# zackLiuzz/MY_ORB_SLAM2

Measured on AMD Instinct MI355X. Metric: frames/sec ORB extract+match, KITTI 1241×376 stereo, 1/2/4/8 GPU, higher is better.
Workload: dtype u8

## Files before the change

### my_orb_slam2_amd/csrc/orbx_capi.hip

```cpp
#include <hip/hip_runtime.h>

#include <algorithm>
#include <chrono>
#include <condition_variable>
#include <cfloat>
#include <climits>
#include <cmath>
#include <cstdio>
#include <cstdlib>
#include <cstring>
#include <functional>
#include <map>
#include <memory>
#include <mutex>
#include <shared_mutex>
#include <thread>
#include <vector>

#include "../../include/orbx.h"
#include "orbx_internal.h"
#include "orbx_kernels.h"

#ifndef ORBX_SRC_HASH
#define ORBX_SRC_HASH "0000000000000000"
// ... 143 lines not shown
        h->sigma2[i] = h->scale[i] * h->scale[i];
    }
    for (int i = 0; i < L; i++) {
        h->inv_scale[i] = 1.0f / h->scale[i];
        h->inv_sigma2[i] = 1.0f / h->sigma2[i];
    }
    const int nfeatures = h->prm.nfeatures;
    float factor = (float)(1.0f / scaleFactor);
    float nDesired = nfeatures * (1 - factor) / (1 - (float)pow((double)factor, (double)L));
    int sum = 0;
    for (int level = 0; level < L - 1; level++) {
        h->nfeat[level] = cvRound(nDesired);
        sum += h->nfeat[level];
        nDesired *= factor;
    }
    h->nfeat[L - 1] = std::max(nfeatures - sum, 0);
    const int HP = 15;
    int v, v0, vmax = cvFloor((float)(HP * std::sqrt(2.f) / 2 + 1));
    int vmin = cvCeil((float)(HP * std::sqrt(2.f) / 2));
    const double hp2 = HP * HP;
    for (v = 0; v <= vmax; ++v) h->umax[v] = cvRound(std::sqrt(hp2 - v * v));
    for (v = HP, v0 = 0; v >= vmin; --v) {
        while (h->umax[v0] == h->umax[v0 + 1]) ++v0;
        h->umax[v] = v0;
        ++v0;
    }
    float cf[7];
    double s2 = -0.5 / (2.0 * 2.0), ksum = 0;
    for (int i = 0; i < 7; ++i) {
        double x = i - 3.0;
        cf[i] = (float)std::exp(s2 * x * x);
        ksum += cf[i];
    }
    ksum = 1. / ksum;
    for (int i = 0; i < 7; ++i) cf[i] = (float)(cf[i] * ksum);
    for (int i = 0; i < 7; ++i) h->taps[i] = cvRound(cf[i] * 256.f);
}

int reflect101_h(int p, int len) {
    if ((unsigned)p < (unsigned)len) return p;
    if (len == 1) return 0;
    do {
        if (p < 0) p = -p;
        else p = 2 * len - 2 - p;
    } while ((unsigned)p >= (unsigned)len);
    return p;
}

void reflected_range_h(int lo, int hi, int len, int& mn, int& mx) {
    mn = 1 << 30;
    mx = -1;
    for (int p = lo; p <= hi; ++p) {
        const int r = reflect101_h(p, len);
        mn = std::min(mn, r);
        mx = std::max(mx, r);
    }
}

int vresize_simd_end(int width) {
    int x = 0;
    for (; x <= width - 16; x += 16) {}
    for (; x < width - 4; x += 4) {}
    return x;
}

static int strip_default(const LevelGeom& lv, int nimg, int ncu) {
    const long long target = 2LL * ncu * 4;
    int th = STRIP_TH;
    while (th > 8 && (long long)lv.snw * ((lv.h + th - 1) / th) * nimg < target) th /= 2;
    return th;
}

static void strip_heights(const orbx_extractor* h, int nimg, int* sth) {
    for (int l = 0; l < ORBX_MAX_LEVELS; ++l) sth[l] = STRIP_TH;
    for (int l = 0; l < h->hg.nlevels; ++l) {
        const LevelGeom& lv = h->hg.lv[l];
        if (lv.strip) sth[l] = strip_default(lv, nimg, h->ncu);
    }
}

static int stereo_split_of(int pairs) { return orbx::stereo_split(pairs); }

#define OCT_LDS_SMALL_KB 152
#define OCT_SMALL_BATCH 16
#define CHAIN_MAX_BATCH 8
#define SIDE_MIN_BATCH 16

static int fast_cells_per_wave(int ncells, int batch, int ncu) {
    int nc = FAST_NC;
    while (nc > 1 && (long long)ncells * batch / (4 * nc) < 2LL * ncu) nc >>= 1;
    return nc;
}

static int octree_small(int batch) { return batch <= OCT_SMALL_BATCH ? 1 : 0; }
static int side_mode_of(const orbx_extractor* h, int batch) {
    return (h->side_auto && batch < SIDE_MIN_BATCH) ? 0 : h->side_mode;
}
static int chain_of(const orbx_extractor* h, int in_place, int side_mode, int batch) {
    return (h->hg.chain_ok && in_place && side_mode == 0 && batch <= CHAIN_MAX_BATCH) ? 1 : 0;
}

static std::shared_mutex g_capture_mu;

static bool order_after_last(orbx_extractor* h, hipStream_t st) {
    if (h->have_done && h->done_stream != st) {
        std::shared_lock<std::shared_mutex> lk(g_capture_mu);
        return HIPOK(hipStreamWaitEvent(st, h->done, 0));
    }
    return true;
}

static bool mark_done(orbx_extractor* h, hipStream_t st) {
    h->done_stream = st;
    h->have_done = true;
    return HIPOK(hipEventRecord(h->done, st));
}

static bool wait_idle(orbx_extractor* h) {
    return !h->have_done || HIPOK(hipEventSynchronize(h->done));
}

#define WAIT_SPIN_US 400
static bool wait_done(orbx_extractor* h) {
    const int spin_us = WAIT_SPIN_US;
    if (spin_us > 0) {
        const auto t0 = std::chrono::steady_clock::now();
        for (;;) {
            const hipError_t e = hipEventQuery(h->done);
            if (e == hipSuccess) return true;
            if (e != hipErrorNotReady) return HIPOK(e);
            if (std::chrono::steady_clock::now() - t0 > std::chrono::microseconds(spin_us)) break;
            std::this_thread::yield();
        }
    }
    return HIPOK(hipEventSynchronize(h->done));
}

static bool ensure_pinned(uint8_t*& p, size_t& cap, size_t n) {
    if (p && cap >= n) return true;
    if (p) (void)hipHostFree(p);
    p = nullptr;
    cap = 0;
    if (!HIPOK(hipHostMalloc((void**)&p, n, hipHostMallocDefault))) { p = nullptr; return false; }
    cap = n;
    return true;
}

void build_strip_tables(orbx_extractor* h, int l, int mode, const int16_t* xofs,
                        const int16_t* alpha, const int16_t* yofs, const int16_t* beta) {
    Geometry& G = h->hg;
    LevelGeom& lv = G.lv[l];
    lv.strip = 0;
    if (mode != 0 && mode != 3) return;
    const LevelGeom& S = G.lv[l > 0 ? l - 1 : 0];
    lv.snh = (lv.w + SW_PX - 1) / SW_PX;
    lv.snw = (lv.snh + 1) / 2;
    std::vector<StripLane> sl((size_t)lv.snh * 32);
    for (int hs = 0; hs < lv.snh; ++hs)
        for (int q = 0; q < 32; ++q) {
            StripLane& e = sl[(size_t)hs * 32 + q];
            memset(&e, 0, sizeof(e));
            int xr[4];
            const int xg = hs * SW_PX - 4 + 4 * q;
            for (int j = 0; j < 4; ++j)
                xr[j] = xg > lv.w + 3 ? lv.w - 1 : reflect101_h(xg + j, lv.w);
            if (mode == 0) {
                const int mn = std::min(std::min(xr[0], xr[1]), std::min(xr[2], xr[3]));
                e.base = (uint32_t)mn;
                for (int j = 0; j < 4; ++j) {
                    if (xr[j] - mn > 4) return;
                    e.sel |= (uint32_t)(xr[j] - mn) << (8 * j);
                }
            } else {
                int sx[4];
                for (int j = 0; j < 4; ++j) sx[j] = xofs[xr[j]];
                const int mn = std::min(std::min(sx[0], sx[1]), std::min(sx[2], sx[3]));
                e.base = (uint32_t)mn;
                for (int j = 0; j < 4; ++j) {
                    const int k = sx[j] - mn;
                    if (k > 6) return;
                    e.psel[j] = (uint32_t)k | (0x0Cu << 8) | ((uint32_t)(k + 1) << 16) | (0x0Cu << 24);
                    uint32_t a0 = (uint16_t)alpha[2 * xr[j]], a1 = (uint16_t)alpha[2 * xr[j] + 1];
                    if (xr[j] >= lv.xmax) { a0 = 2048; a1 = 0; }
                    e.alp[j] = (a0 << 4) | ((a1 << 4) << 16);
                    e.flags |= (uint32_t)((xr[j] < lv.xmax ? 1 : 0) | (xr[j] < lv.rsimd_end ? 2 : 0))
                               << (2 * j);
                }
            }
        }
    std::vector<uint32_t> rt((size_t)4 * (lv.h + 6));
    for (int k = 0; k < lv.h + 6; ++k) {
        const int yr = reflect101_h(k - 3, lv.h);
        if (mode == 0) {
            rt[4 * k] = (uint32_t)yr;
        } else {
            const int sy = yofs[yr];
            const uint32_t r0 = (uint32_t)std::min(std::max(sy, 0), S.h - 1);
            const uint32_t r1 = (uint32_t)std::min(std::max(sy + 1, 0), S.h - 1);
            rt[4 * k] = r0 * (uint32_t)S.pitch;
            rt[4 * k + 1] = r1 * (uint32_t)S.pitch;
            rt[4 * k + 2] = (uint32_t)(uint16_t)beta[2 * yr] | ((uint32_t)(uint16_t)beta[2 * yr + 1] << 16);
        }
    }
    h->ltab.resize(align_up(h->ltab.size(), 16));
    lv.stab = (int)h->ltab.size();
    h->ltab.insert(h->ltab.end(), (const uint8_t*)sl.data(), (const uint8_t*)(sl.data() + sl.size()));
    h->ltab.resize(align_up(h->ltab.size(), 16));
    lv.srow = (int)h->ltab.size();
    h->ltab.insert(h->ltab.end(), (const uint8_t*)rt.data(), (const uint8_t*)(rt.data() + rt.size()));
    h->ltab.resize(align_up(h->ltab.size(), 16));
    lv.strip = 1;
}

static void build_chain(orbx_extractor* h) {
    Geometry& G = h->hg;
    const int L = G.nlevels;
    G.chain_ok = 0;
    G.chain_gx = G.chain_gy = 1;
    G.chain_tab = G.chain_toffs = 0;
    G.chain_buf = G.chain_rs = G.chain_lds = 0;
    for (int l = 1; l < L; ++l) {
        if (G.lv[l].copy || G.lv[l].area2) return;
        const int16_t* xofs = h->rtab.data() + G.lv[l].rtab_off;
        for (int x = 0; x < G.lv[l].w; x += 4)
            if (xofs[std::min(x + 3, G.lv[l].w - 1)] - xofs[x] > 5) return;
    }
    const int gx = std::max(1, (G.lv[0].w + CHAIN_TW - 1) / CHAIN_TW);
    const int gy = std::max(1, (G.lv[0].h + CHAIN_TH - 1) / CHAIN_TH);
    std::vector<ChainRect> rects((size_t)gx * gy * L);
    std::vector<int32_t> toffs((size_t)gx * gy * 2 * (L + 1), 0);
    size_t buf = 16, rs = 16, ct = 16;
    for (int ty = 0; ty < gy; ++ty)
        for (int tx = 0; tx < gx; ++tx) {
            size_t tab = 0;
            bool have_next = false;
            int nx0 = 0, nx1 = -1, ny0 = 0, ny1 = -1;
            for (int l = L - 1; l >= 0; --l) {
                const LevelGeom& lv = G.lv[l];
                const int W = lv.w, Hh = lv.h;
                const int ox0 = tx == 0 ? 0 : ((int)((long long)tx * W / gx) & ~3);
                const int ox1 = std::max(ox0, tx == gx - 1 ? W : ((int)((long long)(tx + 1) * W / gx) & ~3));
                const int oy0 = (int)((long long)ty * Hh / gy);
                const int oy1 = std::max(oy0, ty == gy - 1 ? Hh : (int)((long long)(ty + 1) * Hh / gy));
                int fx0 = INT_MAX, fx1 = -1, fy0 = INT_MAX, fy1 = -1;
                if (ox1 > ox0 && oy1 > oy0) {
                    fx0 = std::max(ox0 - 3, 0);
                    fx1 = std::min(ox1 + 2, W - 1);
                    fy0 = std::max(oy0 - 3, 0);
                    fy1 = std::min(oy1 + 2, Hh - 1);
                }
                if (have_next) {
                    const LevelGeom& D = G.lv[l + 1];
                    const int16_t* xofs = h->rtab.data() + D.rtab_off;
                    const int16_t* yofs = xofs + 3 * D.w;
                    fx0 = std::min(fx0, std::min(std::max((int)xofs[nx0], 0), W - 1));
                    fx1 = std::max(fx1, std::min((int)xofs[nx1] + 1, W - 1));
                    fy0 = std::min(fy0, std::min(std::max((int)yofs[ny0], 0), Hh - 1));
                    fy1 = std::max(fy1, std::min(std::max((int)yofs[ny1] + 1, 0), Hh - 1));
                }
                ChainRect& c = rects[((size_t)ty * gx + tx) * L + l];
                c.ox0 = (int16_t)ox0;
                c.ox1 = (int16_t)ox1;
                c.oy0 = (int16_t)oy0;
                c.oy1 = (int16_t)oy1;
                if (fx1 < 0) {
                    c.fx0 = c.fy0 = 0;
                    c.fx1 = c.fy1 = -1;
                    have_next = false;
                    continue;
                }
                fx0 &= ~3;
                c.fx0 = (int16_t)fx0;
                c.fx1 = (int16_t)fx1;
                c.fy0 = (int16_t)fy0;
                c.fy1 = (int16_t)fy1;
                have_next = true;
                nx0 = fx0;
                nx1 = fx1;
                ny0 = fy0;
                ny1 = fy1;
                const int fw = fx1 - fx0 + 1;
                buf = std::max(buf, (size_t)chain_pitch(fw) * (fy1 - fy0 + 1) + 16);
                rs = std::max(rs, (size_t)4 * ((ox1 - ox0 + 3) & ~3) * (oy1 - oy0 + 6));
                if (l > 0) tab += chain_level_words((fw + 3) >> 2, fy1 - fy0 + 1);
            }
            ct = std::max(ct, 4 * tab);
            int32_t* te = &toffs[((size_t)ty * gx + tx) * 2 * (L + 1)];
            int32_t* tw = te + (L + 1);
            for (int l = 1; l < L; ++l) {
                const ChainRect& c = rects[((size_t)ty * gx + tx) * L + l];
                const int fw = c.fx1 - c.fx0 + 1, fh = c.fy1 - c.fy0 + 1;
                te[l + 1] = te[l] + (fw > 0 ? ((fw + 3) >> 2) + ((fh + 1) & ~1) : 0);
                tw[l + 1] = tw[l] + (fw > 0 ? chain_level_words((fw + 3) >> 2, fh) : 0);
            }
        }
    auto r16 = [](size_t v) { return (v + 15) & ~(size_t)15; };
    const size_t lds = 2 * r16(buf) + r16(rs) + r16(ct);
    if (lds > 150 * 1024) return;
    G.chain_gx = gx;
    G.chain_gy = gy;
    G.chain_buf = (int)r16(buf);
    G.chain_rs = (int)r16(rs);
    G.chain_lds = (int)lds;
    while (h->ltab.size() % 16) h->ltab.push_back(0);
    G.chain_tab = (int)h->ltab.size();
    h->ltab.insert(h->ltab.end(), (const uint8_t*)rects.data(), (const uint8_t*)(rects.data() + rects.size()));
    while (h->ltab.size() % 16) h->ltab.push_back(0);
    G.chain_toffs = (int)h->ltab.size();
    h->ltab.insert(h->ltab.end(), (const uint8_t*)toffs.data(), (const uint8_t*)(toffs.data() + toffs.size()));
    G.chain_ok = 1;
}

orbx_status build_geometry(orbx_extractor* h, int W, int H) {
    Geometry& G = h->hg;
    memset(&G, 0, sizeof(G));
    for (int i = 0; i < 3; ++i)
        if (h->taps[i] != h->taps[6 - i]) return ORBX_ERR_UNSUPPORTED;
    h->cells.clear();
    h->rtab.clear();
    const int L = h->prm.nlevels;
    G.width = W;
    G.height = H;
    G.nlevels = L;
    G.ini_th = std::min(std::max(h->prm.ini_th_fast, 0), 255);
    G.min_th = std::min(std::max(h->prm.min_th_fast, 0), 255);
    memcpy(G.taps, h->taps, sizeof(G.taps));
    memcpy(G.umax, h->umax, sizeof(G.umax));
    for (int l = 0; l < L; ++l)
        G.lv[l].stereo_win = (int)std::ceil(2.0f * h->scale[l]) + 2;
    long long off = 0, cand = 0;
    int out = 0, blur_tiles = 0, oblocks = 0;
    for (int l = 0; l < L; ++l) {
        LevelGeom& lv = G.lv[l];
        lv.w = cvRound((float)W * h->inv_scale[l]);
        lv.h = cvRound((float)H * h->inv_scale[l]);
        if (lv.w <= 0 || lv.h <= 0) return ORBX_ERR_UNSUPPORTED;
        if (lv.w > 4096 + 32 || lv.h > 4096 + 32) return ORBX_ERR_UNSUPPORTED;
        lv.pitch = (int)align_up(lv.w + 4, 64);
        lv.off = off;
        off += (long long)align_up((size_t)lv.pitch * align_up((size_t)lv.h, 4), 256);
        lv.scale = h->scale[l];
        lv.inv_scale = h->inv_scale[l];
        lv.nfeat = h->nfeat[l];
        lv.patch_size = (int)(31 * h->scale[l]);
        const int minB = ORBX_MIN_BORDER;
        const int maxBX = lv.w - ORBX_EDGE + 3, maxBY = lv.h - ORBX_EDGE + 3;
        const float width = (float)(maxBX - minB), height = (float)(maxBY - minB);
        const int nCols = (int)(width / 30.f), nRows = (int)(height / 30.f);
        lv.ncols = nCols;
        lv.nrows = nRows;
        lv.cell_begin = (int)h->cells.size();
        lv.cand_off = cand;
        int lcap = 0;
        if (nCols > 0 && nRows > 0) {
// ... 1522 lines not shown
```

### my_orb_slam2_amd/csrc/orbx_pyramid.hip

```cpp
#include <hip/hip_runtime.h>
#include <stdint.h>

#include <type_traits>
#include <utility>

#include "orbx_device.h"
#include "orbx_internal.h"
#include "orbx_kernels.h"

namespace orbx {


#define LT_GW (LT_W / 4)

__device__ __forceinline__ int reflect101_i(int p, int len) {
    if ((unsigned)p < (unsigned)len) return p;
    if (len == 1) return 0;
    do {
        if (p < 0) p = -p;
        else p = 2 * len - 2 - p;
    } while ((unsigned)p >= (unsigned)len);
    return p;
}

// ... 380 lines not shown
            const uint32_t wa0 = __builtin_amdgcn_alignbyte(a1, a0, o0);
            const uint32_t wa1 = __builtin_amdgcn_alignbyte(a2, a1, o0);
            const uint32_t wc0 = __builtin_amdgcn_alignbyte(c1, c0, o0);
            const uint32_t wc1 = __builtin_amdgcn_alignbyte(c2, c1, o0);
            const bool all_simd = FASTP || ((ci >> 1) & 0x55u) == 0x55u;
            auto hsum = [&](int j, int& h0, int& h1) {
                const uint32_t p0 = __builtin_amdgcn_perm(wa1, wa0, sels[j]);
                const uint32_t p1 = __builtin_amdgcn_perm(wc1, wc0, sels[j]);
                const us2 al = __builtin_bit_cast(us2, als[j]);
                h0 = (int)__builtin_amdgcn_udot2(__builtin_bit_cast(us2, p0), al, 0u, false);
                h1 = (int)__builtin_amdgcn_udot2(__builtin_bit_cast(us2, p1), al, 0u, false);
            };
            const uint32_t bs0 = (uint32_t)b0 << 8, bs1 = (uint32_t)b1 << 8;
            auto mulhi24 = [](uint32_t x, uint32_t y) {
                return (uint32_t)(((uint64_t)(x & 0xFFFFFFu) * (y & 0xFFFFFFu)) >> 32);
            };
            auto vsimd = [&](int H0, int H1) {
                return (int)((mulhi24((uint32_t)H0 & ~0xFFu, bs0) +
                              mulhi24((uint32_t)H1 & ~0xFFu, bs1) + 2u) >> 2);
            };
            if (all_simd) {
#pragma unroll
                for (int j = 0; j < 4; ++j) {
                    int h0, h1;
                    hsum(j, h0, h1);
                    out |= (uint32_t)vsimd(h0, h1) << (8 * j);
                }
            } else {
#pragma unroll
                for (int j = 0; j < 4; ++j) {
                    int h0, h1;
                    hsum(j, h0, h1);
                    const int vs = vsimd(h0, h1);
                    h0 >>= 4;
                    h1 >>= 4;
                    const int vc = min((int)((__umul24(h0, b0) + __umul24(h1, b1) + (1u << 21)) >> 22), 255);
                    out |= (uint32_t)(((ci >> (2 * j + 1)) & 1u) ? vs : vc) << (8 * j);
                }
            }
        } else {
#pragma unroll
            for (int j = 0; j < 4; ++j) {
                const int sxj = xs[j];
                const int f = (int)(ci >> (2 * j)) & 3;
                int h0, h1;
                if (f & 1) {
                    const int aa = (int)(int16_t)(als[j] & 0xFFFF), ab = (int)(int16_t)(als[j] >> 16);
                    h0 = w0[sxj] * aa + w0[sxj + 1] * ab;
                    h1 = w1[sxj] * aa + w1[sxj + 1] * ab;
                } else {
                    h0 = w0[sxj] * 2048;
                    h1 = w1[sxj] * 2048;
                }
                out |= (uint32_t)vresize(h0, h1, b0, b1, (f & 2) != 0) << (8 * j);
            }
        }
        return out;
    };
    auto level_item = [&](int hr, int q, bool all) {
        const int y = Y0 - 3 + hr, xg = X0 - 4 + 4 * q;
        uint32_t out = 0;
        if (all || (y >= ny0 && y <= ny1 && xg + 3 >= nx0 && xg <= nx1)) {
            const uint2 cg = cgrp[q];
            const uint32_t ci = cinf[q];
            const uint2 ri = rinf[hr];
            const int xs[4] = {(int)(cg.x & 0xFFFF), (int)(cg.x >> 16), (int)(cg.y & 0xFFFF),
                               (int)(cg.y >> 16)};
            if (mode == 3) {
                out = item3(hr, cg, ci, calp[q], csel[q], std::false_type{});
            } else if (mode == 2) {
                const int yr = (int)ri.x;
#pragma unroll
                for (int j = 0; j < 4; ++j) {
                    const uint8_t* s0 = src2 + (size_t)(2 * yr) * S.pitch + 2 * xs[j];
                    out |= (uint32_t)((s0[0] + s0[1] + s0[S.pitch] + s0[S.pitch + 1] + 2) >> 2) << (8 * j);
                }
            } else {
                const uint8_t* wr = win + __umul24(ri.x & 0xFFFF, WP);
                if (ci & 0x100u) {
                    out = *(const uint32_t*)(wr + xs[0]);
                } else {
                    out = (uint32_t)wr[xs[0]] | ((uint32_t)wr[xs[1]] << 8) |
                          ((uint32_t)wr[xs[2]] << 16) | ((uint32_t)wr[xs[3]] << 24);
                }
            }
        }
        lvl[hr * LT_G + q] = out;
    };
    if (!direct && mode == 3 && full_tile) {
        if (tid < 7 * LT_G) {
            const int rs = (int)(__umul24((uint32_t)tid, 1928u) >> 16);
            const int q = tid - rs * LT_G;
            const uint2 cg = cgrp[q];
            const uint32_t ci = cinf[q];
            const uint4 al = calp[q], sl = csel[q];
            const bool fast = (ci & 0x200u) && ((ci >> 1) & 0x55u) == 0x55u;
            if (__all(fast)) {
#pragma unroll
                for (int k = 0; k < (LT_HR + 6) / 7; ++k) {
                    const int hr = rs + 7 * k;
                    if (hr < LT_HR) lvl[hr * LT_G + q] = item3(hr, cg, ci, al, sl, std::true_type{});
                }
            } else {
#pragma unroll
                for (int k = 0; k < (LT_HR + 6) / 7; ++k) {
                    const int hr = rs + 7 * k;
                    if (hr < LT_HR) lvl[hr * LT_G + q] = item3(hr, cg, ci, al, sl, std::false_type{});
                }
            }
        }
    } else
    if (!direct) {
        int hr = tid / LT_G, q = tid - hr * LT_G;
        if (full_tile) {
            constexpr int KF = (LT_HR * LT_G) / 256, RF = (LT_HR * LT_G) % 256;
#pragma unroll
            for (int k = 0; k < KF; ++k) {
                level_item(hr, q, true);
                hr += 7;
                q += 18;
                if (q >= LT_G) { q -= LT_G; ++hr; }
            }
            if (tid < RF) level_item(hr, q, true);
        } else {
            for (int i = tid; i < LT_HR * LT_G;
                 i += 256, hr += 7, q += 18, (q >= LT_G ? (q -= LT_G, ++hr) : 0))
                level_item(hr, q, false);
        }
    }
    __syncthreads();

    uint8_t* dlev = pyr + (size_t)b * g->pyr_bytes + L.off;
    uint8_t* dblur = blur + (size_t)b * g->pyr_bytes + L.off;
    const int k0 = g->taps[0], k1 = g->taps[1], k2 = g->taps[2], k3 = g->taps[3];
    const int k4 = g->taps[4], k5 = g->taps[5], k6 = g->taps[6];
    const BlurTaps tp = {(uint32_t)k0 | (uint32_t)k1 << 8 | (uint32_t)k2 << 16 | (uint32_t)k3 << 24,
                         (uint32_t)k4 | (uint32_t)k5 << 8 | (uint32_t)k6 << 16,
                         (uint32_t)k4 * 0x10001u, (uint32_t)k5 * 0x10001u, (uint32_t)k6 * 0x10001u,
                         (uint32_t)k3};
    const bool full = vw == LT_W && vh == LT_H;
    float* rowsf = (float*)rows;
    if (full) tile_out_rows_f<true>(lvl, rowsf, tid, vw, vh, dlev, X0, Y0, L.pitch, tp);
    else tile_out_rows_f<false>(lvl, rowsf, tid, vw, vh, dlev, X0, Y0, L.pitch, tp);
    __syncthreads();
    if (full) tile_columns_f<true>(rowsf, tid, vw, vh, dblur, X0, Y0, L.pitch, L.h, L.bsimd_end, tp);
    else tile_columns_f<false>(rowsf, tid, vw, vh, dblur, X0, Y0, L.pitch, L.h, L.bsimd_end, tp);
}

#define STRIP_PF 2
#define STRIP_ST_POLICY 0
#define STRIP_LEV rlev
#define STRIP_HREUSE 1
#define STRIP_HMASK 1
#define STRIP_SYNC0 0
#define STRIP_SYNC3 2
#define STRIP_SYNC_LEVELS 0xFFFF
#define STRIP_NS3 2
#define STRIP_NS0 7
#define STRIP_PF0 6
typedef unsigned int v4u __attribute__((ext_vector_type(4)));
typedef unsigned int v3u __attribute__((ext_vector_type(3)));
template <typename F, int... K>
__device__ __forceinline__ void unroll_seq(F&& f, std::integer_sequence<int, K...>) {
    (f(std::integral_constant<int, K>{}), ...);
}
#define STRIP_WPE0 6
#define STRIP_WPE3 5
template <int MODE>
__device__ __forceinline__ void level_strip_wave(const Geometry* __restrict__ g,
                                                 const uint8_t* __restrict__ ltab,
                                                 const uint8_t* __restrict__ in0,
                                                 const uint8_t* __restrict__ in1, int split,
                                                 size_t stride, size_t bstride,
                                                 uint8_t* __restrict__ pyr,
                                                 uint8_t* __restrict__ blur, int level, int sth,
                                                 int sync, int wv, int b, uint32_t* sbl) {
    static_assert(MODE == 0 || MODE == 3 || MODE == 4, "strip kernel: level 0 or INTER_LINEAR levels");
    constexpr bool L0 = MODE != 3;
    const int lane = threadIdx.x & 63, half = lane >> 5, l32 = lane & 31;
    const LevelGeom& L = g->lv[level];
    const int sns = (L.h + sth - 1) / sth;
    if (wv >= L.snw * sns) return;
    const int swx = wv % L.snw, sy = wv / L.snw;
    const int hs = 2 * swx + half;
    const bool hvalid = hs < L.snh;
    const int hsc = min(hs, L.snh - 1);
    const int W = L.w, H = L.h, pitch = L.pitch;
    const int x = hsc * SW_PX - 4 + 4 * l32;
    const int Y0 = sy * sth, vh = min(sth, H - Y0);
    const bool out_lane = hvalid && l32 >= 1 && l32 <= SW_OUT && x < W;
    const StripLane* T = (const StripLane*)(ltab + L.stab) + hsc * 32 + l32;
    const uint4 t0 = *(const uint4*)T;
    const uint4 al = *(const uint4*)T->alp;
    const uint4 ps = *(const uint4*)T->psel;
    const uint4* RT = (const uint4*)(ltab + L.srow) + Y0;
    const int n = vh + 6;

    const uint8_t* src;
    size_t spitch;
    if (MODE == 4) {
        src = pyr + (size_t)b * g->pyr_bytes + L.off;
        spitch = (size_t)pitch;
    } else if (MODE == 0) {
        src = b < split ? in0 + (size_t)b * bstride : in1 + (size_t)(b - split) * bstride;
        spitch = stride;
    } else {
        const LevelGeom& S = g->lv[level - 1];
        src = pyr + (size_t)b * g->pyr_bytes + S.off;
        spitch = (size_t)S.pitch;
    }
    const __amdgpu_buffer_rsrc_t rsrc = __builtin_amdgcn_make_buffer_rsrc((void*)src, 0, 0x7FFFFFFF, 0x00020000);
    const uint32_t o0 = t0.x & 3u;
    const uint32_t boff = t0.x & ~3u;
    const uint32_t xoff4 = t0.x + 4u;

    const bool lane_rsimd = ((t0.y >> 1) & 0x55u) == 0x55u;
    const bool wave_rsimd = __all(!hvalid || lane_rsimd);
    const bool wave_bsimd = __all(!out_lane || x + 4 <= L.bsimd_end);

    const BlurTaps tp = {(uint32_t)g->taps[0] | (uint32_t)g->taps[1] << 8 | (uint32_t)g->taps[2] << 16 |
                             (uint32_t)g->taps[3] << 24,
                         (uint32_t)g->taps[4] | (uint32_t)g->taps[5] << 8 | (uint32_t)g->taps[6] << 16,
                         0u, 0u, 0u, (uint32_t)g->taps[3]};
    const float inv = 1.0f / 65536.0f;
    const float f3 = (float)g->taps[3] * inv, f4 = (float)g->taps[4] * inv,
                f5 = (float)g->taps[5] * inv, f6 = (float)g->taps[6] * inv;
    const uint32_t k0 = g->taps[0], k1 = g->taps[1], k2 = g->taps[2], k3 = g->taps[3],
                   k4 = g->taps[4], k5 = g->taps[5], k6 = g->taps[6];
    const uint32_t W00 = k0 << 8 | k1 << 16 | k2 << 24, W01 = k3 | k4 << 8 | k5 << 16 | k6 << 24;
    const uint32_t W10 = k0 << 16 | k1 << 24, W11 = k2 | k3 << 8 | k4 << 16 | k5 << 24, W12 = k6;
    const uint32_t W20 = k0 << 24, W21 = k1 | k2 << 8 | k3 << 16 | k4 << 24, W22 = k5 | k6 << 8;
    (void)W00; (void)W01; (void)W10; (void)W11; (void)W12; (void)W20; (void)W21; (void)W22;

    auto row_info = [&](int i) { return RT[i]; };
    constexpr int NS = L0 ? STRIP_NS0 : STRIP_NS3;
    constexpr int PF = L0 ? STRIP_PF0 : STRIP_PF;
    static_assert(PF <= NS && (NS == 1 || NS == 2 || NS == 3 || NS == 7), "slot ring");
    uint32_t A[NS][3], C[NS][3], RB[NS];
    uint32_t RAo[NS], RCo[NS], HCp[4] = {0u, 0u, 0u, 0u};
    uint32_t prevRC = 0xFFFFFFFFu;
    auto issue = [&](int slot, int i) {
        const int ic = min(i, n - 1);
        const uint4 ri = row_info(ic);
        if (L0) {
            const uint8_t* rowp = src + (size_t)(ri.x & 0xFFFFu) * spitch;
            const uint32_t rlo = (uint32_t)(uintptr_t)rowp - 4u;
            const uint32_t o = (rlo + xoff4) & 3u;
            const uint32_t aoff = xoff4 - o;
            const uint32_t last = ((rlo + 4u + (uint32_t)(W - 1)) & ~3u) - rlo;
            A[slot][0] = *(const uint32_t*)(rowp + aoff - 4);
            A[slot][1] = *(const uint32_t*)(rowp + min(aoff + 4u, last) - 4);
            A[slot][2] = t0.z + __builtin_amdgcn_perm(0u, o, 0u);
        } else {
            const v3u a3 = __builtin_bit_cast(v3u, __builtin_amdgcn_raw_buffer_load_b96(rsrc, boff, ri.x, 0));
            const v3u c3 = __builtin_bit_cast(v3u, __builtin_amdgcn_raw_buffer_load_b96(rsrc, boff, ri.y, 0));
            A[slot][0] = a3.x; A[slot][1] = a3.y; A[slot][2] = a3.z;
            C[slot][0] = c3.x; C[slot][1] = c3.y; C[slot][2] = c3.z;
            RB[slot] = ri.z;
            RAo[slot] = ri.x;
            RCo[slot] = ri.y;
        }
    };
    auto mulhi24 = [](uint32_t a, uint32_t c) {
        return (uint32_t)(((uint64_t)(a & 0xFFFFFFu) * (c & 0xFFFFFFu)) >> 32);
    };
    auto level_group = [&](int slot, auto simd_c) -> uint32_t {
        if (L0) return __builtin_amdgcn_perm(A[slot][1], A[slot][0], A[slot][2]);
        constexpr bool SIMD = decltype(simd_c)::value;
        const uint32_t rb = RB[slot];
        const int b0 = (int)(int16_t)(rb & 0xFFFF), b1 = (int)(int16_t)(rb >> 16);
        const uint32_t bs0 = (uint32_t)b0 << 8, bs1 = (uint32_t)b1 << 8;
        const uint32_t sels[4] = {ps.x, ps.y, ps.z, ps.w};
        const uint32_t als[4] = {al.x, al.y, al.z, al.w};
        auto hrow = [&](const uint32_t* D, uint32_t* hs) {
            const uint32_t w0 = __builtin_amdgcn_alignbyte(D[1], D[0], o0);
            const uint32_t w1 = __builtin_amdgcn_alignbyte(D[2], D[1], o0);
#pragma unroll
            for (int j = 0; j < 4; ++j) {
                hs[j] = __builtin_amdgcn_udot2(__builtin_bit_cast(us2, __builtin_amdgcn_perm(w1, w0, sels[j])),
                                               __builtin_bit_cast(us2, als[j]), 0u, false);
                if (SIMD && STRIP_HMASK) hs[j] &= ~0xFFu;
            }
        };
        uint32_t hA[4], hC[4];
        if (RAo[slot] == prevRC) {
#pragma unroll
            for (int j = 0; j < 4; ++j) hA[j] = HCp[j];
        } else {
            hrow(A[slot], hA);
        }
        hrow(C[slot], hC);
#pragma unroll
        for (int j = 0; j < 4; ++j) HCp[j] = hC[j];
        prevRC = RCo[slot];
        uint32_t out = 0;
#pragma unroll
        for (int j = 0; j < 4; ++j) {
            int h0 = (int)hA[j];
            int h1 = (int)hC[j];
            const uint32_t hm = (SIMD && STRIP_HMASK) ? ~0u : ~0xFFu;
            const int vs = (int)((mulhi24((uint32_t)h0 & hm, bs0) +
                                  mulhi24((uint32_t)h1 & hm, bs1) + 2u) >> 2);
            if (SIMD) {
                out |= (uint32_t)vs << (8 * j);
            } else {
                h0 >>= 4;
                h1 >>= 4;
                const int vc = min((int)((__umul24(h0, b0) + __umul24(h1, b1) + (1u << 21)) >> 22), 255);
                out |= (uint32_t)(((t0.y >> (2 * j + 1)) & 1u) ? vs : vc) << (8 * j);
            }
        }
        return out;
    };
    float4 R[7];
    uint8_t* const lev0 = pyr + (size_t)b * g->pyr_bytes + L.off;
    uint8_t* const blr0 = blur + (size_t)b * g->pyr_bytes + L.off;
    const int nrec = pitch * H;
    const __amdgpu_buffer_rsrc_t rlev = __builtin_amdgcn_make_buffer_rsrc(lev0, 0, nrec, 0x00020000);
    const __amdgpu_buffer_rsrc_t rblr = __builtin_amdgcn_make_buffer_rsrc(blr0, 0, pitch * ((H + 3) & ~3), 0x00020000);
    const uint32_t lane_off = out_lane ? (uint32_t)x : 0x80000000u;
    auto store_row = [&](const __amdgpu_buffer_rsrc_t& rs, int r, bool ok, uint32_t v) {
        __builtin_amdgcn_raw_buffer_store_b32(v, rs, ok ? lane_off : 0x80000000u, ok ? r * pitch : 0, STRIP_ST_POLICY);
    };
    const int sbl_dw = (l32 >= 1 && l32 <= SW_OUT) ? SW_OUT * half + l32 - 1 : 60;
    const int ft = lane % 15, fj = lane / 15;
    const int ftx = 15 * (wv % L.snw) + ft;
    const uint32_t fl_off = (lane < 60 && 16 * ftx < W) ? (uint32_t)(64 * ftx + 16 * fj) : 0x80000000u;
    auto step = [&](auto k_c, int i, auto rsimd_c, auto bsimd_c, auto all_c) __attribute__((always_inline)) {
        constexpr int k = decltype(k_c)::value;
        constexpr bool ALL = decltype(all_c)::value;
        constexpr bool BSIMD = decltype(bsimd_c)::value;
        __builtin_amdgcn_sched_barrier(0);
        const uint32_t v = level_group(k % NS, rsimd_c);
        issue((k + PF) % NS, i + PF);
        if constexpr (MODE != 4) store_row(STRIP_LEV, Y0 + i - 3, ALL || (i >= 3 && i < vh + 3), v);
        const uint32_t d0 = (uint32_t)__builtin_amdgcn_update_dpp(0, (int)v, 0x138, 0xF, 0xF, true);
        const uint32_t d2 = (uint32_t)__builtin_amdgcn_update_dpp(0, (int)v, 0x130, 0xF, 0xF, true);
        float4 o;
        auto dot4 = [](uint32_t a, uint32_t w, uint32_t c) { return __builtin_amdgcn_udot4(a, w, c, false); };
        o.x = (float)dot4(d0, W00, dot4(v, W01, 0u));
        o.y = (float)dot4(d0, W10, dot4(v, W11, dot4(d2, W12, 0u)));
        o.z = (float)dot4(d0, W20, dot4(v, W21, dot4(d2, W22, 0u)));
        o.w = (float)dot4(v, tp.tapA, dot4(d2, tp.tapB, 0u));
        R[k % 7] = o;
        {
            auto r = [&](int t) -> const float4& { return R[(k - t + 14) % 7]; };
            float S[4];
#pragma unroll
            for (int hp = 0; hp < 2; ++hp) {
                auto c = [&](int t) {
                    const float4& q = r(t);
                    return hp == 0 ? f2v{q.x, q.y} : f2v{q.z, q.w};
                };
                const f2v F6 = {f6, f6}, F5 = {f5, f5}, F4 = {f4, f4}, F3 = {f3, f3};
                f2v a = (c(6) + c(0)) * F6;
                a = __builtin_elementwise_fma(c(5) + c(1), F5, a);
                a = __builtin_elementwise_fma(c(4) + c(2), F4, a);
                a = __builtin_elementwise_fma(c(3), F3, a);
                S[2 * hp] = a.x;
                S[2 * hp + 1] = a.y;
            }
            uint32_t packed = 0;
            if (BSIMD) {
#pragma unroll
                for (int j = 0; j < 4; ++j) packed = __builtin_amdgcn_cvt_pk_u8_f32(S[j], j, packed);
            } else {
#pragma unroll
                for (int j = 0; j < 4; ++j) {
                    const uint32_t Si = (uint32_t)(S[j] * 65536.0f);
                    const bool simd = x + j < L.bsimd_end;
                    const uint32_t val = (Si + (simd ? 32767u + ((Si >> 16) & 1u) : 32768u)) >> 16;
                    packed |= min(val, 255u) << (8 * j);
                }
            }
            const int slot = (i + 2) & 3;
            sbl[slot * 64 + sbl_dw] = packed;
            if (slot == 3) {
                __builtin_amdgcn_fence(__ATOMIC_SEQ_CST, "wavefront");
                const uint32_t* fp = (const uint32_t*)__builtin_assume_aligned(sbl + 64 * fj + 4 * ft, 16);
                const v4u q = {fp[0], fp[1], fp[2], fp[3]};
                const bool ok = ALL || (i >= 9 && i - 9 < vh);
                __builtin_amdgcn_raw_buffer_store_b128(q, rblr, ok ? fl_off : 0x80000000u,
                                                       ok ? (Y0 + i - 9) * pitch : 0, STRIP_ST_POLICY);
                __asm__ volatile("s_nop 4" ::"v"(q));
                __builtin_amdgcn_fence(__ATOMIC_SEQ_CST, "wavefront");
            }
        }
    };
    constexpr int U = NS == 7 ? 7 : 7 * NS;
    auto walk = [&](auto rsimd_c, auto bsimd_c) __attribute__((always_inline)) {
#pragma unroll
        for (int i = 0; i < PF; ++i) {
            issue(i % NS, i);
            if constexpr (MODE != 4) store_row(STRIP_LEV, 0, false, 0u);
        }
        int nblk = 0;
        auto block = [&](int i0, auto all_c) __attribute__((always_inline)) {
            if (sync > 0) {
                if (nblk % sync == 0) __builtin_amdgcn_s_barrier();
                ++nblk;
            }
            unroll_seq([&](auto k_c) { step(k_c, i0 + decltype(k_c)::value, rsimd_c, bsimd_c, all_c); },
                       std::make_integer_sequence<int, U>{});
        };
        int i0 = 0;
        static_assert(U >= 6, "the first block holds the halo steps");
        block(0, std::false_type{});
        for (i0 = U; i0 + U <= vh + 3; i0 += U) block(i0, std::true_type{});
        const int nend = ((vh + 3) & ~3) + 6;
        for (; i0 < nend; i0 += U) block(i0, std::false_type{});
    };
    if ((L0 || wave_rsimd) && wave_bsimd) walk(std::true_type{}, std::true_type{});
    else walk(std::false_type{}, std::false_type{});
}

template <int MODE>
__global__ __launch_bounds__(512) __attribute__((amdgpu_waves_per_eu(MODE != 3 ? STRIP_WPE0 : STRIP_WPE3))) void k_level_strip(const Geometry* __restrict__ g,
                                                     const uint8_t* __restrict__ ltab,
                                                     const uint8_t* __restrict__ in0,
                                                     const uint8_t* __restrict__ in1, int split,
                                                     size_t stride, size_t bstride,
                                                     uint8_t* __restrict__ pyr,
                                                     uint8_t* __restrict__ blur, int level,
                                                     int sth, int sync) {
    int bx, b;
    xcd_block(bx, b);
    const int wv = bx * (int)(blockDim.x >> 6) + __builtin_amdgcn_readfirstlane((int)(threadIdx.x >> 6));
    __shared__ __attribute__((aligned(16))) uint32_t sbl[8][4 * 64];
    level_strip_wave<MODE>(g, ltab, in0, in1, split, stride, bstride, pyr, blur, level, sth, sync,
                           wv, b, sbl[threadIdx.x >> 6]);
}

#define CHAIN_NT 1024
__device__ __forceinline__ int reflect101_fast(int p, int len) {
    return (unsigned)p < (unsigned)len ? p : reflect101_i(p, len);
}

__device__ __forceinline__ uint32_t mulhi_u24(uint32_t x, uint32_t y) {
    return (uint32_t)(((uint64_t)(x & 0xFFFFFFu) * (y & 0xFFFFFFu)) >> 32);
}

__device__ __forceinline__ uint32_t x_simd_bits(int x0, int x1, int rsimd_end) {
    uint32_t m = 0;
#pragma unroll
    for (int j = 0; j < 4; ++j) m |= (min(x0 + j, x1) < rsimd_end ? 1u : 0u) << j;
    return m;
}

struct Div {
    uint32_t m, d;
    __device__ explicit Div(int dd) : m(dd > 1 ? 0xFFFFFFFFu / (uint32_t)dd + 1u : 0u), d((uint32_t)dd) {}
    __device__ int operator()(int i) const { return d > 1 ? (int)__umulhi((uint32_t)i, m) : i; }
};

template <int NT>
__device__ __forceinline__ bool chain_fill(const ChainRect& c, const LevelGeom& Lv, uint8_t* buf,
                                           int P, int tid) {
    const int W = Lv.w, fh = c.fy1 - c.fy0 + 1;
    const bool left = c.fx0 == 0, right = c.fx1 == W - 1;
    if (!left && !right) return false;
    for (int i = tid; i < 2 * fh; i += NT) {
        const int r = i >> 1;
        uint8_t* row = buf + r * P + 4 - c.fx0;
        if ((i & 1) == 0 && left) {
            row[-1] = row[min(1, W - 1)];
            row[-2] = row[reflect101_fast(-2, W)];
            row[-3] = row[reflect101_fast(-3, W)];
        } else if ((i & 1) == 1 && right) {
            row[W] = row[reflect101_fast(W, W)];
            row[W + 1] = row[reflect101_fast(W + 1, W)];
            row[W + 2] = row[reflect101_fast(W + 2, W)];
        }
    }
    return true;
}

template <int NT>
__device__ __forceinline__ void chain_rows(const ChainRect& c, const LevelGeom& Lv, const uint8_t* src,
                                           int P, int* rsum, const Geometry* g, int tid) {
    const int ow = c.ox1 - c.ox0, oh = c.oy1 - c.oy0;
    if (ow <= 0 || oh <= 0) return;
    const int ng = (ow + 3) >> 2, RW = 4 * ng;
    const int H = Lv.h;
    const uint32_t tapA = (uint32_t)g->taps[0] | (uint32_t)g->taps[1] << 8 | (uint32_t)g->taps[2] << 16 |
                          (uint32_t)g->taps[3] << 24;
    const uint32_t tapB = (uint32_t)g->taps[4] | (uint32_t)g->taps[5] << 8 | (uint32_t)g->taps[6] << 16;
    const Div dv(ng);
    for (int i = tid; i < (oh + 6) * ng; i += NT) {
        const int rr = dv(i), q = i - rr * ng;
        const int ry = reflect101_fast(c.oy0 - 3 + rr, H) - c.fy0;
        const int xg = c.ox0 + 4 * q;
        const uint32_t* sw = (const uint32_t*)(src + ry * P + (xg - c.fx0));
        const uint32_t d0 = sw[0], d1 = sw[1], d2 = sw[2];
        int4 o;
        o.x = (int)__builtin_amdgcn_udot4(__builtin_amdgcn_alignbyte(d1, d0, 1), tapA,
                  __builtin_amdgcn_udot4(__builtin_amdgcn_alignbyte(d2, d1, 1), tapB, 0u, false), false);
        o.y = (int)__builtin_amdgcn_udot4(__builtin_amdgcn_alignbyte(d1, d0, 2), tapA,
                  __builtin_amdgcn_udot4(__builtin_amdgcn_alignbyte(d2, d1, 2), tapB, 0u, false), false);
        o.z = (int)__builtin_amdgcn_udot4(__builtin_amdgcn_alignbyte(d1, d0, 3), tapA,
                  __builtin_amdgcn_udot4(__builtin_amdgcn_alignbyte(d2, d1, 3), tapB, 0u, false), false);
        o.w = (int)__builtin_amdgcn_udot4(d1, tapA, __builtin_amdgcn_udot4(d2, tapB, 0u, false), false);
        *(int4*)(rsum + rr * RW + 4 * q) = o;
    }
}

template <int NT>
__device__ __forceinline__ void chain_cols(const ChainRect& c, const LevelGeom& Lv, const int* rsum,
                                           uint8_t* dblur, const Geometry* g, int tid) {
    const int ow = c.ox1 - c.ox0, oh = c.oy1 - c.oy0;
    if (ow <= 0 || oh <= 0) return;
    const int ng = (ow + 3) >> 2, RW = 4 * ng;
    const uint32_t t3 = (uint32_t)g->taps[3], t4 = (uint32_t)g->taps[4];
    const uint32_t t5 = (uint32_t)g->taps[5], t6 = (uint32_t)g->taps[6];
    const Div dv(ng);
    for (int i = tid; i < oh * ng; i += NT) {
        const int rr = dv(i), q = i - rr * ng;
        const int y = c.oy0 + rr, xg = c.ox0 + 4 * q;
        int4 v[7];
#pragma unroll
        for (int k = 0; k < 7; ++k) v[k] = *(const int4*)(rsum + (rr + k) * RW + 4 * q);
        uint32_t packed = 0;
#pragma unroll
        for (int j = 0; j < 4; ++j) {
            auto e = [&](int k) { return (uint32_t)((const int*)&v[k])[j]; };
            const uint32_t S = t3 * e(3) + t4 * (e(2) + e(4)) + t5 * (e(1) + e(5)) + t6 * (e(0) + e(6));
            const bool simd = xg + j < Lv.bsimd_end;
            const uint32_t val = (S + (simd ? 32767u + ((S >> 16) & 1u) : 32768u)) >> 16;
            packed |= min(val, 255u) << (8 * j);
        }
        uint8_t* d = dblur + blur_off(xg, y, Lv.pitch, Lv.h);
        if (xg + 4 <= c.ox1) *(uint32_t*)d = packed;
        else
            for (int j = 0; xg + j < c.ox1; ++j) d[j] = (uint8_t)(packed >> (8 * j));
    }
}


template <int NT>
__global__ __launch_bounds__(NT) void k_pyr_chain(const Geometry* __restrict__ g,
                                                  const uint8_t* __restrict__ ltab,
                                                  const int16_t* __restrict__ rtab,
                                                  uint8_t* __restrict__ pyr,
                                                  uint8_t* __restrict__ blur) {
    extern __shared__ __attribute__((aligned(16))) uint8_t smem[];
    const int tile = blockIdx.x, b = blockIdx.y;
    const int tid = threadIdx.x;
// ... 264 lines not shown
```

Baseline: 137,000.

## Skip redundant row loads, prefetch row table, use b64 level-0 loads in strip kernel

The row table now carries a flag marking rows whose first source row equals the previous row's second source row. The strip kernel uses that flag to push the buffer load out of range, so the redundant load is skipped and the cached horizontal result is reused. Row-table entries are prefetched one step ahead for the resize levels. Level 0 in mode 4 switches to a single 64-bit buffer load, guarded host-side by an alignment check on offset and pitch. These changes cut redundant global loads and address arithmetic, but add more table state and a fallback path when alignment fails.

```diff
diff --git a/my_orb_slam2_amd/csrc/orbx_capi.hip b/my_orb_slam2_amd/csrc/orbx_capi.hip
--- a/my_orb_slam2_amd/csrc/orbx_capi.hip
+++ b/my_orb_slam2_amd/csrc/orbx_capi.hip
@@ -319,6 +319,7 @@
     LevelGeom& lv = G.lv[l];
     lv.strip = 0;
     if (mode != 0 && mode != 3) return;
+    if (mode == 0 && ((lv.off | lv.pitch) & 3) != 0) return;
     const LevelGeom& S = G.lv[l > 0 ? l - 1 : 0];
     lv.snh = (lv.w + SW_PX - 1) / SW_PX;
     lv.snw = (lv.snh + 1) / 2;
@@ -367,6 +368,7 @@
             rt[4 * k] = r0 * (uint32_t)S.pitch;
             rt[4 * k + 1] = r1 * (uint32_t)S.pitch;
             rt[4 * k + 2] = (uint32_t)(uint16_t)beta[2 * yr] | ((uint32_t)(uint16_t)beta[2 * yr + 1] << 16);
+            rt[4 * k + 3] = (k > 0 && rt[4 * k] == rt[4 * k - 3]) ? 0x80000000u : 0u;
         }
     }
     h->ltab.resize(align_up(h->ltab.size(), 16));
diff --git a/my_orb_slam2_amd/csrc/orbx_pyramid.hip b/my_orb_slam2_amd/csrc/orbx_pyramid.hip
--- a/my_orb_slam2_amd/csrc/orbx_pyramid.hip
+++ b/my_orb_slam2_amd/csrc/orbx_pyramid.hip
@@ -556,6 +556,9 @@
 #define STRIP_LEV rlev
 #define STRIP_HREUSE 1
 #define STRIP_HMASK 1
+#define STRIP_AVOID 1
+#define STRIP_RTPF 1
+#define STRIP_L0B64 1
 #define STRIP_SYNC0 0
 #define STRIP_SYNC3 2
 #define STRIP_SYNC_LEVELS 0xFFFF
@@ -564,6 +567,7 @@
 #define STRIP_PF0 6
 typedef unsigned int v4u __attribute__((ext_vector_type(4)));
 typedef unsigned int v3u __attribute__((ext_vector_type(3)));
+typedef unsigned int v2u __attribute__((ext_vector_type(2)));
 template <typename F, int... K>
 __device__ __forceinline__ void unroll_seq(F&& f, std::integer_sequence<int, K...>) {
     (f(std::integral_constant<int, K>{}), ...);
@@ -641,12 +645,24 @@
     constexpr int PF = L0 ? STRIP_PF0 : STRIP_PF;
     static_assert(PF <= NS && (NS == 1 || NS == 2 || NS == 3 || NS == 7), "slot ring");
     uint32_t A[NS][3], C[NS][3], RB[NS];
-    uint32_t RAo[NS], RCo[NS], HCp[4] = {0u, 0u, 0u, 0u};
-    uint32_t prevRC = 0xFFFFFFFFu;
-    auto issue = [&](int slot, int i) {
+    uint32_t RAr[NS], HCp[4] = {0u, 0u, 0u, 0u};
+    uint4 rnext = {0u, 0u, 0u, 0u};
+    if (!L0 && STRIP_RTPF) rnext = row_info(0);
+    auto issue = [&](int slot, int i, bool first) {
         const int ic = min(i, n - 1);
-        const uint4 ri = row_info(ic);
-        if (L0) {
+        uint4 ri;
+        if (!L0 && STRIP_RTPF) {
+            ri = rnext;
+            rnext = row_info(min(i + 1, n - 1));
+        } else {
+            ri = row_info(ic);
+        }
+        if (MODE == 4 && STRIP_L0B64) {
+            const v2u a2 = __builtin_bit_cast(v2u, __builtin_amdgcn_raw_buffer_load_b64(
+                rsrc, boff, (ri.x & 0xFFFFu) * (uint32_t)pitch, 0));
+            A[slot][0] = a2.x; A[slot][1] = a2.y;
+            A[slot][2] = t0.z + __builtin_amdgcn_perm(0u, o0, 0u);
+        } else if (L0) {
             const uint8_t* rowp = src + (size_t)(ri.x & 0xFFFFu) * spitch;
             const uint32_t rlo = (uint32_t)(uintptr_t)rowp - 4u;
             const uint32_t o = (rlo + xoff4) & 3u;
@@ -656,13 +672,13 @@
             A[slot][1] = *(const uint32_t*)(rowp + min(aoff + 4u, last) - 4);
             A[slot][2] = t0.z + __builtin_amdgcn_perm(0u, o, 0u);
         } else {
-            const v3u a3 = __builtin_bit_cast(v3u, __builtin_amdgcn_raw_buffer_load_b96(rsrc, boff, ri.x, 0));
+            const uint32_t rep = (!first && i < n) ? ri.w : 0u;
+            const v3u a3 = __builtin_bit_cast(v3u, __builtin_amdgcn_raw_buffer_load_b96(rsrc, STRIP_AVOID ? boff | rep : boff, ri.x, 0));
             const v3u c3 = __builtin_bit_cast(v3u, __builtin_amdgcn_raw_buffer_load_b96(rsrc, boff, ri.y, 0));
             A[slot][0] = a3.x; A[slot][1] = a3.y; A[slot][2] = a3.z;
             C[slot][0] = c3.x; C[slot][1] = c3.y; C[slot][2] = c3.z;
             RB[slot] = ri.z;
-            RAo[slot] = ri.x;
-            RCo[slot] = ri.y;
+            RAr[slot] = rep;
         }
     };
     auto mulhi24 = [](uint32_t a, uint32_t c) {
@@ -687,7 +703,7 @@
             }
         };
         uint32_t hA[4], hC[4];
-        if (RAo[slot] == prevRC) {
+        if (RAr[slot] != 0u) {
 #pragma unroll
             for (int j = 0; j < 4; ++j) hA[j] = HCp[j];
         } else {
@@ -696,7 +712,6 @@
         hrow(C[slot], hC);
 #pragma unroll
         for (int j = 0; j < 4; ++j) HCp[j] = hC[j];
-        prevRC = RCo[slot];
         uint32_t out = 0;
 #pragma unroll
         for (int j = 0; j < 4; ++j) {
@@ -736,7 +751,7 @@
         constexpr bool BSIMD = decltype(bsimd_c)::value;
         __builtin_amdgcn_sched_barrier(0);
         const uint32_t v = level_group(k % NS, rsimd_c);
-        issue((k + PF) % NS, i + PF);
+        issue((k + PF) % NS, i + PF, false);
         if constexpr (MODE != 4) store_row(STRIP_LEV, Y0 + i - 3, ALL || (i >= 3 && i < vh + 3), v);
         const uint32_t d0 = (uint32_t)__builtin_amdgcn_update_dpp(0, (int)v, 0x138, 0xF, 0xF, true);
         const uint32_t d2 = (uint32_t)__builtin_amdgcn_update_dpp(0, (int)v, 0x130, 0xF, 0xF, true);
@@ -795,7 +810,7 @@
     auto walk = [&](auto rsimd_c, auto bsimd_c) __attribute__((always_inline)) {
 #pragma unroll
         for (int i = 0; i < PF; ++i) {
-            issue(i % NS, i);
+            issue(i % NS, i, i == 0);
             if constexpr (MODE != 4) store_row(STRIP_LEV, 0, false, 0u);
         }
         int nblk = 0;
```

Measured after the change: 138,100, median of 6. Within noise of the previous version (+0.8%).
